# ElesionKyrie/Extreme-Video-Compression-With-Prediction-Using-Pre-trainded-Diffusion-Models-

Measured on AMD Instinct MI355X. Metric: decoded frames/sec (128x128x30) at q3, higher is better.
Workload: dtype f32

## Files before the change

extreme-video-compression-with-prediction-using-pre-trainded-diffusion-models-_amd/build.py:

```python
import os
import shutil
import subprocess
import sys
from concurrent.futures import ThreadPoolExecutor

HERE = os.path.dirname(os.path.abspath(__file__))
CSRC = os.path.join(HERE, "csrc")
LIBDIR = os.path.join(HERE, "lib")
OBJDIR = os.path.join(HERE, "build")
INCLUDE = os.path.join(os.path.dirname(HERE), "include")
HIP_SOURCES = ["conv_igemm.hip", "attention.hip", "norm.hip", "fir.hip", "elementwise.hip", "gdn.hip", "stride2.hip", "lpips.hip", "i3d.hip", "frames.hip", "noise.hip", "yuv.hip", "rate.hip", "ssim.hip", "metric.hip", "inception.hip", "resample.hip", "tile.hip", "api.hip"]
ARCH = "gfx950"


def _newer(target, deps):
    if not os.path.exists(target):
        return True
    t = os.path.getmtime(target)
    return any(os.path.getmtime(d) > t for d in deps)


def _run(cmd):
    r = subprocess.run(cmd, capture_output=True, text=True)
    if r.returncode != 0:
        raise RuntimeError("build failed: %s\n%s\n%s" % (" ".join(cmd), r.stdout, r.stderr))


def hipcc_path():
    for c in (os.environ.get("HIPCC"), shutil.which("hipcc"), "/opt/rocm/bin/hipcc"):
        if c and os.path.exists(c):
            return c
    raise RuntimeError("hipcc not found (ROCm toolchain required to build libevc_hip.so)")


def build(force=False, verbose=False):
    os.makedirs(LIBDIR, exist_ok=True)
    os.makedirs(OBJDIR, exist_ok=True)
    headers = [os.path.join(INCLUDE, h) for h in ("evc_hip.h", "evc_rans.h")]
    hipcc = hipcc_path()
    flags = ["--offload-arch=" + ARCH, "-O3", "-std=c++17", "-fPIC", "-I", INCLUDE]
    flags += os.environ.get("EVC_HIPCC_FLAGS", "").split()

    def compile_one(src):
        s = os.path.join(CSRC, src)
        o = os.path.join(OBJDIR, src.replace(".hip", ".o"))
        if force or _newer(o, [s] + headers):
            if verbose:
                print("hipcc", src, flush=True)
            _run([hipcc] + flags + ["-c", s, "-o", o])
        return o

    with ThreadPoolExecutor(max_workers=min(6, len(HIP_SOURCES))) as ex:
        objs = list(ex.map(compile_one, HIP_SOURCES))
    hip_so = os.path.join(LIBDIR, "libevc_hip.so")
    if force or _newer(hip_so, objs):
        _run([hipcc, "--offload-arch=" + ARCH, "-shared", "-fPIC", "-o", hip_so] + objs)
    rans_src = os.path.join(CSRC, "rans.cpp")
    rans_so = os.path.join(LIBDIR, "libevc_rans.so")
    if force or _newer(rans_so, [rans_src] + headers):
        _run([shutil.which("g++") or "g++", "-O2", "-std=c++17", "-fPIC", "-shared", "-Wall", "-I", INCLUDE,
              rans_src, "-o", rans_so])
# ... 6 lines not shown
```

extreme-video-compression-with-prediction-using-pre-trainded-diffusion-models-_amd/csrc/conv_igemm.hip:

```cpp
#include <hip/hip_runtime.h>
#include <stdint.h>
#include <stdio.h>
#include "../../include/evc_hip.h"

typedef float f32x16 __attribute__((ext_vector_type(16)));
typedef __attribute__((address_space(3))) void lds_void;
typedef const __attribute__((address_space(1))) void glb_void;

#ifndef EVC_CONV_TAIL
#define EVC_CONV_TAIL 1
#endif
#ifndef EVC_CONV_TM1
#define EVC_CONV_TM1 1
#endif
#ifndef EVC_SPLIT_WIDE_TILES
#define EVC_SPLIT_WIDE_TILES 1
#endif

#ifndef EVC_SPLIT_INTERLEAVE
#define EVC_SPLIT_INTERLEAVE 5
#endif

namespace {

constexpr int BM_MAX = 128;
constexpr int KC = 16;

constexpr int MODE_PLAIN = 0, MODE_AFFINE = 1, MODE_AFFINE_SILU = 2, MODE_SILU = 3, MODE_RELU = 4;

struct ConvK {
    const float* src0; const float* src1; int C0; int C1; int ld0; int ld1;
    const float* coef_a; const float* coef_s;
    const float* w; const float* bias; const float* res; int ld_res;
    float out_scale; int act_out;
    float* out; int ld_out;
    int B, H, W, Co, CoPad, KH, KW;
    int M, HW, nchunk, nsteps, steps_per_split, splits;
    float* ws;
    float* stats;
    const float* w_hdr;
    const unsigned* in_bound;
    int tail_first, tail_splits, tail_sps, tail_rows;
    int cut_chunk;
    const float* x2_src0; const float* x2_src1; int x2_C0, x2_C1, x2_ld0, x2_ld1;
    const char* x2_w;
    const float* x2_hdr;
    const unsigned* x2_bound;
    int bound_stride, generic_epi;
};

__device__ __forceinline__ float bound_scale(unsigned bits) {
    const float b = sqrtf(__uint_as_float(bits));
    if (!(b < 3.0e38f)) return __builtin_nanf("");
    return b > 0.f ? ldexpf(1.0f, 6 - ilogbf(b)) : 1.0f;
}
__device__ __forceinline__ int bound_index(const ConvK& p, int m) { return p.bound_stride ? min(m, p.M - 1) / p.HW : 0; }
__device__ __forceinline__ float in_scale(const ConvK& p, int m) {
    if (!p.in_bound) return 1.0f;
    return bound_scale(p.in_bound[bound_index(p, m)]);
}

__device__ __forceinline__ float silu_f(float v) { return v * __builtin_amdgcn_rcpf(1.0f + __expf(-v)); }

__device__ __forceinline__ float act_fn(float v, int act) {
    if (act == EVC_ACT_SILU) return silu_f(v);
    if (act == EVC_ACT_RELU) return v < 0.f ? 0.f : v;
    return v;
}

template <int MODE>
__device__ __forceinline__ float4 transform(float4 v, const float4& a, const float4& s, bool ok) {
    if (MODE == MODE_AFFINE || MODE == MODE_AFFINE_SILU) {
        v.x = v.x * a.x + s.x; v.y = v.y * a.y + s.y; v.z = v.z * a.z + s.z; v.w = v.w * a.w + s.w;
    }
    if (MODE == MODE_AFFINE_SILU || MODE == MODE_SILU) {
        v.x = silu_f(v.x); v.y = silu_f(v.y); v.z = silu_f(v.z); v.w = silu_f(v.w);
    }
    if (MODE == MODE_RELU) {
// ... 248 lines not shown
        issue_loads(buf ^ 1);

        const float* Ab = As + buf * BM * KC + a_rd;
        const float* Wb = Ws + buf * BN * KC + w_rd;
        float4 a0[TM], b0[TN], a1[TM], b1[TN];
#pragma unroll
        for (int i = 0; i < TM; ++i) a0[i] = *reinterpret_cast<const float4*>(Ab + i * 32 * KC + rd0);
#pragma unroll
        for (int j = 0; j < TN; ++j) b0[j] = *reinterpret_cast<const float4*>(Wb + j * 32 * KC + rd0);
#pragma unroll
        for (int i = 0; i < TM; ++i) a1[i] = *reinterpret_cast<const float4*>(Ab + i * 32 * KC + rd1);
#pragma unroll
        for (int j = 0; j < TN; ++j) b1[j] = *reinterpret_cast<const float4*>(Wb + j * 32 * KC + rd1);
        mfma_group<TM, TN>(acc, a0, b0);
        __builtin_amdgcn_sched_barrier(0);
        store_a(buf ^ 1);
        mfma_group<TM, TN>(acc, a1, b1);
        __syncthreads();
    }

    conv_epilogue<TM, TN>(p, acc, m0, n0, split, wm, wn, l31, half);
}

typedef __bf16 bf16x8 __attribute__((ext_vector_type(8)));
typedef _Float16 f16x8 __attribute__((ext_vector_type(8)));

__device__ __forceinline__ void split3_bf16(const float4& v0, const float4& v1, bf16x8& p1, bf16x8& p2, bf16x8& p3) {
    const float x[8] = {v0.x, v0.y, v0.z, v0.w, v1.x, v1.y, v1.z, v1.w};
#pragma unroll
    for (int j = 0; j < 8; ++j) {
        const __bf16 a = (__bf16)x[j];
        const float r = x[j] - (float)a;
        const __bf16 b = (__bf16)r;
        p1[j] = a; p2[j] = b; p3[j] = (__bf16)(r - (float)b);
    }
}

constexpr float F16_ACT_SCALE = 8.0f;

__device__ __forceinline__ void split2_f16(const float4& v0, const float4& v1, float xscale, f16x8& p1, f16x8& p2) {
    const float x[8] = {v0.x, v0.y, v0.z, v0.w, v1.x, v1.y, v1.z, v1.w};
#pragma unroll
    for (int j = 0; j < 8; ++j) {
        const float v = x[j] * xscale;
        const _Float16 a = (_Float16)v;
        p1[j] = a; p2[j] = (_Float16)(v - (float)a);
    }
}

template <int NP> struct Split;
template <> struct Split<3> {
    typedef bf16x8 vec;
    static constexpr int NTERM = 6;
    static __device__ __forceinline__ constexpr int qa(int t) { return t == 0 ? 2 : (t == 1 || t == 3) ? 1 : 0; }
    static __device__ __forceinline__ constexpr int qb(int t) { return t == 2 ? 2 : (t == 1 || t == 4) ? 1 : 0; }
    static __device__ __forceinline__ f32x16 mfma(const vec& a, const vec& b, const f32x16& c) {
        return __builtin_amdgcn_mfma_f32_32x32x16_bf16(a, b, c, 0, 0, 0);
    }
    static __device__ __forceinline__ void split(const float4& v0, const float4& v1, float, vec (&pl)[3]) {
        split3_bf16(v0, v1, pl[0], pl[1], pl[2]);
    }
};
template <> struct Split<2> {
    typedef f16x8 vec;
    static constexpr int NTERM = 3;
    static __device__ __forceinline__ constexpr int qa(int t) { return t == 0 ? 1 : 0; }
    static __device__ __forceinline__ constexpr int qb(int t) { return t == 1 ? 1 : 0; }
    static __device__ __forceinline__ f32x16 mfma(const vec& a, const vec& b, const f32x16& c) {
        return __builtin_amdgcn_mfma_f32_32x32x16_f16(a, b, c, 0, 0, 0);
    }
    static __device__ __forceinline__ void split(const float4& v0, const float4& v1, float xscale, vec (&pl)[2]) {
        split2_f16(v0, v1, xscale, pl[0], pl[1]);
    }
};

template <int NP, int TM, int TN, int MODE>
__global__ __launch_bounds__(256, 2) void conv_splitn_kernel(ConvK p) {
    typedef Split<NP> SP;
    typedef typename SP::vec vec;
    constexpr int BM = 64 * TM;
    constexpr int BN = 64 * TN;
    constexpr int RB = 32;
    constexpr int NPIECE = NP * 2 * TN;
    constexpr int NWD = (NPIECE + 3) / 4;
    constexpr bool HAS_COEF = MODE == MODE_AFFINE || MODE == MODE_AFFINE_SILU;
    extern __shared__ __attribute__((aligned(16))) char smem_b[];
    char* const As = smem_b;
    char* const Ws = smem_b + 2 * NP * BM * RB;

    const int tid = threadIdx.x;
    const int lane = tid & 63;
    const int wave = __builtin_amdgcn_readfirstlane(tid >> 6);
    const int wm = wave >> 1, wn = wave & 1;
    const int l31 = lane & 31, half = lane >> 5;

    const int m0 = blockIdx.x * BM;
    const int n0 = blockIdx.y * BN;
// ... 1196 lines not shown
__global__ void conv_pack_split_kernel(const float* w, __bf16* packed, int Co, int CoPad, int Ci, int KH, int KW) {
    const int taps = KH * KW, nchunk = Ci / KC;
    const size_t total = (size_t)taps * nchunk * CoPad * KC;
    for (size_t i = (size_t)blockIdx.x * blockDim.x + threadIdx.x; i < total; i += (size_t)gridDim.x * blockDim.x) {
        const int k = (int)(i % KC);
        size_t t = i / KC;
        const int co = (int)(t % CoPad); t /= CoPad;
        const int chunk = (int)(t % nchunk);
        const int tap = (int)(t / nchunk);
        float v = 0.f;
        if (co < Co) v = w[((size_t)co * Ci + chunk * KC + k) * taps + tap];
        const __bf16 a = (__bf16)v;
        const float r = v - (float)a;
        const __bf16 b = (__bf16)r;
        const __bf16 c = (__bf16)(r - (float)b);
        const int pos = (((k >> 3) ^ ((co >> 3) & 1)) << 3) | (k & 7);
        const size_t base = (size_t)(tap * nchunk + chunk) * 3 * CoPad * KC;
        packed[base + ((size_t)0 * CoPad + co) * KC + pos] = a;
        packed[base + ((size_t)1 * CoPad + co) * KC + pos] = b;
        packed[base + ((size_t)2 * CoPad + co) * KC + pos] = c;
    }
}

constexpr int F16_HDR_BYTES = 256;

__global__ void conv_absmax_kernel(const float* w, size_t n, unsigned* out_bits) {
    float m = 0.f;
    for (size_t i = (size_t)blockIdx.x * blockDim.x + threadIdx.x; i < n; i += (size_t)gridDim.x * blockDim.x)
        m = fmaxf(m, fabsf(w[i]));
    for (int o = 32; o > 0; o >>= 1) m = fmaxf(m, __shfl_xor(m, o));
    if ((threadIdx.x & 63) == 0 && m > 0.f) atomicMax(out_bits, __float_as_uint(m));
}

__device__ __forceinline__ float f16_weight_scale(unsigned max_bits) {
    const float mx = __uint_as_float(max_bits);
    if (!(mx > 0.f) || !isfinite(mx)) return 1.0f;
    return ldexpf(1.0f, 14 - ilogbf(mx));
}

__global__ void conv_pack_f16_kernel(const float* w, char* packed, int Co, int CoPad, int Ci, int KH, int KW) {
    const int taps = KH * KW, nchunk = Ci / KC;
    const size_t total = (size_t)taps * nchunk * CoPad * KC;
    float* hdr = reinterpret_cast<float*>(packed);
    const float sw = f16_weight_scale(reinterpret_cast<const unsigned*>(packed)[2]);
    _Float16* body = reinterpret_cast<_Float16*>(packed + F16_HDR_BYTES);
    if (blockIdx.x == 0 && threadIdx.x == 0) { hdr[0] = 1.0f / (F16_ACT_SCALE * sw); hdr[1] = sw; }
    for (size_t i = (size_t)blockIdx.x * blockDim.x + threadIdx.x; i < total; i += (size_t)gridDim.x * blockDim.x) {
// ... 585 lines not shown
```

extreme-video-compression-with-prediction-using-pre-trainded-diffusion-models-_amd/lib.py:

```python
import ctypes
import math
import os
from ctypes import POINTER, c_char_p, c_double, c_float, c_int, c_int32, c_longlong, c_uint, c_uint8, c_ulonglong, c_void_p

import numpy as np
import torch

HERE = os.path.dirname(os.path.abspath(__file__))
HIP_SO = os.path.join(HERE, "lib", "libevc_hip.so")
if os.environ.get("EVC_HIP_SO"):
    HIP_SO = os.path.abspath(os.environ["EVC_HIP_SO"])
RANS_SO = os.path.join(HERE, "lib", "libevc_rans.so")

ACT_NONE, ACT_SILU, ACT_RELU = 0, 1, 2
ARITH_F32, ARITH_BF16X6, ARITH_F16X3 = 0, 1, 2
_ARITH_NAMES = {"f32": ARITH_F32, "bf16x6": ARITH_BF16X6, "f16x3": ARITH_F16X3}
_ARITH_DTYPES = {ARITH_F32: torch.float32, ARITH_BF16X6: torch.bfloat16, ARITH_F16X3: torch.float16}


def _arith_policy():
    name = os.environ.get("EVC_CONV_ARITH", "f16x3").lower()
    if name not in _ARITH_NAMES:
        raise ValueError(f"EVC_CONV_ARITH must be one of {sorted(_ARITH_NAMES)}, got {name!r}")
    return _ARITH_NAMES[name]
# ... 13 lines not shown


class EvcKernelError(RuntimeError):
    pass


class ConvArgs(ctypes.Structure):
    _fields_ = [("src0", c_void_p), ("src1", c_void_p), ("C0", c_int), ("C1", c_int),
                ("ld0", c_int), ("ld1", c_int),
                ("coef_a", c_void_p), ("coef_s", c_void_p), ("act_in", c_int),
                ("w_packed", c_void_p), ("bias", c_void_p), ("res", c_void_p), ("ld_res", c_int),
                ("out_scale", c_float), ("act_out", c_int),
                ("out", c_void_p), ("ld_out", c_int),
                ("B", c_int), ("H", c_int), ("W", c_int), ("Co", c_int), ("KH", c_int), ("KW", c_int),
                ("splits", c_int), ("stats_out", c_void_p), ("arith", c_int), ("in_bound", c_void_p),
                ("x2_src0", c_void_p), ("x2_src1", c_void_p), ("x2_C0", c_int), ("x2_C1", c_int), ("x2_ld0", c_int),
                ("x2_ld1", c_int), ("x2_w_packed", c_void_p), ("x2_bound", c_void_p), ("invariant", c_int)]


class ConvPlan(ctypes.Structure):
    _fields_ = [("kernel", ctypes.c_char * 96), ("tile_m", c_int), ("tile_n", c_int), ("splits", c_int),
                ("steps_per_split", c_int), ("cut_chunk", c_int), ("tail_tiles", c_int), ("tail_splits", c_int),
                ("stats_runs", c_int), ("fused_1x1", c_int)]


class AttentionPlan(ctypes.Structure):
    _fields_ = [("kernel", ctypes.c_char * 64), ("waves", c_int), ("kparts", c_int), ("tiles_per_part", c_int),
                ("kv_planes", c_int), ("merge", c_int), ("short_seq", c_int),
                ("lds_bytes", c_longlong), ("parts_bytes", c_longlong), ("ws_bytes", c_longlong)]


HIP_SYMBOLS = {
    "evc_version": (c_char_p, []),
    "evc_arch": (c_char_p, []),
    "evc_device_ok": (c_int, []),
    "evc_clock_probe": (c_int, [c_void_p, c_int, c_void_p, c_void_p]),
    "evc_im2col_nchw_f32": (c_int, [c_void_p, c_void_p] + [c_int] * 9 + [c_void_p, c_void_p, c_void_p]),
    "evc_maxpool3s2_nhwc_f32": (c_int, [c_void_p, c_void_p, c_int, c_int, c_int, c_int, c_void_p]),
    "evc_lpips_layer_f32": (c_int, [c_void_p, c_void_p, c_void_p, c_void_p, c_int, c_int, c_int, c_int, c_void_p]),
    "evc_maxpool2d_nhwc_f32": (c_int, [c_void_p, c_void_p] + [c_int] * 7 + [c_void_p]),
    "evc_lpips_map_f32": (c_int, [c_void_p, c_void_p, c_void_p, c_void_p, c_int, c_int, c_int, c_void_p]),
    "evc_lpips_map_mean_f32": (c_int, [c_void_p, c_void_p, c_int, c_int, c_int, c_void_p]),
    "evc_lpips_upsample_add_f32": (c_int, [c_void_p, c_void_p] + [c_int] * 6 + [c_void_p]),
    "evc_i3d_stem_im2col_f32": (c_int, [c_void_p, c_void_p] + [c_int] * 17 + [c_void_p]),
    "evc_maxpool3d_same_nthwc_f32": (c_int, [c_void_p, c_void_p] + [c_int] * 11 + [c_void_p]),
    "evc_i3d_head_f32": (c_int, [c_void_p] * 4 + [c_int] * 6 + [c_void_p]),
# ... 39 lines not shown
    "evc_deconv5x5s2_f32": (c_int, [c_void_p, c_void_p, c_int, c_void_p, c_void_p, c_void_p] + [c_int] * 6 + [c_void_p]),
    "evc_conv5x5s2_workspace_bytes": (c_longlong, [c_int, c_int, c_int, c_int]),
    "evc_conv5x5s2_f32": (c_int, [c_void_p, c_int, c_void_p, c_int, c_void_p, c_void_p, c_void_p] + [c_int] * 6 + [c_void_p]),
    "evc_gdn_workspace_bytes": (c_longlong, [c_int, c_int, c_int, c_int]),
    "evc_gdn_f32": (c_int, [c_void_p, c_void_p, c_int, c_void_p, c_void_p, c_void_p, c_int, c_int, c_int, c_int, c_int,
                            c_int, c_void_p]),
    "evc_affine_act_nhwc_f32": (c_int, [c_void_p, c_void_p, c_void_p, c_void_p, c_int, c_int, c_int, c_int, c_int,
                                        c_int, c_void_p]),
    "evc_conv_co_pad": (c_int, [c_int]),
    "evc_conv_packed_floats": (c_longlong, [c_int, c_int, c_int, c_int]),
    "evc_conv_pack_weights_f32": (c_int, [c_void_p, c_void_p, c_int, c_int, c_int, c_int, c_void_p]),
    "evc_conv_packed_bytes": (c_longlong, [c_int, c_int, c_int, c_int, c_int]),
    "evc_conv_pack_weights": (c_int, [c_void_p, c_void_p, c_int, c_int, c_int, c_int, c_int, c_void_p]),
    "evc_conv_set_option": (c_int, [c_char_p, c_int]),
    "evc_spade_act_nhwc_f32": (c_int, [c_void_p, c_void_p, c_void_p, c_void_p, c_int, c_void_p, c_void_p, c_int, c_void_p,
                                       c_void_p, c_int, c_void_p, c_int, c_int, c_int, c_int, c_int, c_void_p]),
    "evc_conv_choose_splits": (c_int, [POINTER(ConvArgs)]),
    "evc_conv_kernel_name": (c_int, [POINTER(ConvArgs), c_char_p, c_int]),
    "evc_conv_fused_1x1_supported": (c_int, [POINTER(ConvArgs)]),
    "evc_conv_stats_splits": (c_int, [POINTER(ConvArgs)]),
    "evc_conv_workspace_bytes": (c_longlong, [POINTER(ConvArgs)]),
    "evc_conv2d_nhwc_f32": (c_int, [POINTER(ConvArgs), c_void_p, c_void_p]),
    "evc_conv2d_nhwc_profiled_f32": (c_int, [POINTER(ConvArgs), c_void_p, c_void_p, c_void_p, c_void_p]),
    "evc_attention_f32": (c_int, [c_void_p, c_void_p, c_void_p, c_int, c_void_p, c_int, c_int, c_int, c_int, c_int,
                                  c_float, c_void_p]),
    "evc_attention_workspace_bytes": (c_longlong, [c_int, c_int, c_int, c_int]),
    "evc_attention_set_option": (c_int, [c_char_p, c_int]),
    "evc_attention_plan_query": (c_int, [c_int, c_int, c_int, c_int, c_int, c_int, c_int, POINTER(AttentionPlan)]),
    "evc_attention_ws_f32": (c_int, [c_void_p, c_void_p, c_void_p, c_int, c_void_p, c_int, c_int, c_int, c_int, c_int,
                                     c_float, c_void_p, c_void_p]),
    "evc_frame_group_norm_f32": (c_int, [c_void_p] * 4 + [c_int] * 5 + [c_float, c_void_p]),
    "evc_frame_attention_f32": (c_int, [c_void_p, c_int, c_void_p, c_int] + [c_int] * 5 + [c_float, c_void_p]),
    "evc_frame_mix_f32": (c_int, [c_void_p] * 4 + [c_int] * 3 + [c_longlong, c_void_p]),
    "evc_frame_taps_f32": (c_int, [c_void_p, c_void_p] + [c_int] * 4 + [c_void_p]),
    "evc_ddpm_step_f32": (c_int, [c_void_p, c_void_p, c_void_p, c_longlong] + [c_float] * 5 + [c_int, c_void_p]),
    "evc_ddim_step_f32": (c_int, [c_void_p, c_void_p, c_longlong] + [c_float] * 4 + [c_int, c_void_p]),
    "evc_axpy_f32": (c_int, [c_void_p, c_void_p, c_void_p, c_longlong, c_float, c_void_p]),
    "evc_pndm_transfer_f32": (c_int, [c_void_p, c_void_p, c_void_p, c_longlong, c_float, c_float, c_float, c_int,
                                      c_void_p]),
    "evc_lincomb4_f32": (c_int, [c_void_p] * 5 + [c_longlong] + [c_float] * 4 + [c_void_p]),
    "evc_scale_clamp_f32": (c_int, [c_void_p, c_void_p, c_longlong, c_float, c_float, c_int, c_float, c_float,
                                    c_void_p]),
    "evc_gate_residual_f32": (c_int, [c_void_p, c_void_p, c_void_p, c_void_p, c_longlong, c_void_p]),
    "evc_elic_gather_params_f32": (c_int, [c_void_p] + [c_int] * 8 + [c_void_p, c_int, c_void_p, c_void_p,
                                                                       c_void_p]),
    "evc_elic_scatter_symbols_f32": (c_int, [c_void_p, c_void_p, c_void_p] + [c_int] * 7 + [c_void_p]),
# ... 669 lines not shown
                                 shape=(B, H, W, C0 + C1, Co, KH),
                                 call=dict(B=B, H=H, W=W, C0=C0, C1=C1, Co=Co, K=KH, coef=coef is not None, act_in=act_in,
                                           res=res is not None, out_scale=float(out_scale), bias=bias is not None,
                                           bound=in_bound is not None, arith=a.arith, ld_out=ldo,
                                           stats=bool(want_stats), x2=x2_ci, invariant=inv)))
    else:
        _check(L.evc_conv2d_nhwc_f32(ctypes.byref(a), ptr(ws), stream_ptr()), "evc_conv2d_nhwc_f32")
    result = out.t if isinstance(out, Cols) else out
    if want_stats:
        return result, (stats if stats is not None else chan_stats(result, invariant=inv))
    return result


def conv_fused_stats_splits(B, H, W, Ci, Co, KH, KW, splits=0, arith=None):
    a = conv_query_args(B, H, W, Ci, 0, Co, KH, KW, default_arith() if arith is None else arith, splits=splits)
    return hip_lib(require_device=False).evc_conv_stats_splits(ctypes.byref(a))


def conv_workspace_bytes(B, H, W, Ci, Co, KH, KW, splits=0, arith=None):
    a = conv_query_args(B, H, W, Ci, 0, Co, KH, KW, default_arith() if arith is None else arith, splits=splits)
    return hip_lib(require_device=False).evc_conv_workspace_bytes(ctypes.byref(a))


def attention_set_option(name, value):
    if hip_lib(require_device=False).evc_attention_set_option(name.encode(), int(value)) != 0:
        raise EvcKernelError(f"unknown attention option {name!r}")


ATTN_PROFILE = None


def attention_plan(B, heads, N, D, with_bounds=False, have_ws=None, invariant=False):
    L = hip_lib(require_device=False)
    if have_ws is None:
        nbytes = (L.evc_attention_invariant_workspace_bytes if invariant else L.evc_attention_workspace_bytes)(B, heads, N, D)
        have_ws = nbytes > 0
    out = AttentionPlan()
    _check(L.evc_attention_plan_query(B, heads, N, D, int(bool(with_bounds)), int(bool(have_ws)), int(bool(invariant)),
                                      ctypes.byref(out)), "evc_attention_plan_query")
    return dict(kernel=out.kernel.decode(), waves=out.waves, kparts=out.kparts, tiles_per_part=out.tiles_per_part,
                kv_planes=bool(out.kv_planes), merge=bool(out.merge), short_seq=bool(out.short_seq),
                lds_bytes=out.lds_bytes, parts_bytes=out.parts_bytes, ws_bytes=out.ws_bytes)


def attention(qkv, C, heads, out=None, bounds=None, invariant=False, ws=None):
    L = hip_lib()
# ... 536 lines not shown
```

extreme-video-compression-with-prediction-using-pre-trainded-diffusion-models-_amd/scorenet.py:

```python
import math
from types import SimpleNamespace

import numpy as np
import torch

from . import lib as L

FIR_K = np.outer([1, 3, 3, 1], [1, 3, 3, 1]).astype(np.float32)
FIR_K /= FIR_K.sum()
INV_SQRT2 = float(np.float32(1.0) / np.sqrt(np.float32(2.0)))


def num_groups(ch):
    g = min(ch // 4, 32)
    while ch % g != 0:
        g -= 1
    return g


def dims_from_config(config):
    m, d = config.model, config.data
    return SimpleNamespace(ngf=m.ngf, ch_mult=list(m.ch_mult), num_res_blocks=m.num_res_blocks,
                           attn_resolutions=list(m.attn_resolutions), n_head_channels=m.n_head_channels,
                           image_size=d.image_size, channels=d.channels, num_frames=d.num_frames,
# ... 492 lines not shown
        else:
            torch.cuda.current_stream().wait_event(done)
        if fuse:
            x2 = (xs, None, e["w2"], xbound) if xs is not None else (x.t, s1, e["w2"], xbound)
            return self._act(*self._conv(h1.t, e["w1"], m["cout"], 3, 3, bias=e["b12"], coef=coef1, act_in=L.ACT_SILU,
                                       out_scale=INV_SQRT2, want_stats=True, x2=x2))
        if self.preactivate:
            h1a = L.affine_act(h1.t, coef1, L.ACT_SILU)
            return self._act(*self._conv(h1a, e["w1"], m["cout"], 3, 3, bias=e["b1"], res=xs, out_scale=INV_SQRT2,
                                       want_stats=True))
        return self._act(*self._conv(h1.t, e["w1"], m["cout"], 3, 3, bias=e["b1"], coef=coef1, act_in=L.ACT_SILU,
                                   res=xs, out_scale=INV_SQRT2, want_stats=True))

    def _attn(self, i, m, x):
        e = self.w[i]
        B, H, W, C = x.t.shape
        hd = self.d.n_head_channels
        heads = 1 if C < hd else C // hd
        coef = self._gn([x.stats()], H * W, num_groups(C), 1e-6, mode=1, gamma=e["gamma"], beta=e["beta"],
                           site=self._site("attn_norm", i))
        qkvb = self._bound_slot(3)
        if qkvb is None:
            obound = None
            qkv = self._conv(x.t, e["wqkv"], 3 * C, 1, 1, bias=e["bqkv"], coef=coef)
        else:
            qkv, qst = self._conv(x.t, e["wqkv"], 3 * C, 1, 1, bias=e["bqkv"], coef=coef, want_stats=True)
            self._mbound(qst, 0, C, qkvb, site=self._site("attn_qkv", i))
            obound = _f16_only(e["wo"], qkvb.view(B, 3)[:, 2].contiguous() if self.batch_invariant else qkvb[2:3])
        o = self._attention(qkv.view(B, H * W, 3 * C), C, heads, bounds=None if i in self._attn_f32 else qkvb)
        return self._act(*self._conv(o.view(B, H, W, C), e["wo"], C, 1, 1, bias=e["bo"], res=x.t,
                                   out_scale=INV_SQRT2, want_stats=True, in_bound=obound))

    @torch.no_grad()
    def forward_rows(self, x, rows, cond=None):
        if self.batch_invariant and self._demoted:
            raise ValueError("batch-invariant mode does not combine with demoted sites (range recovery)")
        return self._forward_rows(x, rows, cond)

    def _forward_rows(self, x, rows, cond=None):
        d = self.d
        prog = self.program
        B, _, H, W = x.shape
        self._bound_batch = B if self.batch_invariant else 1
        nb = 256 * self._bound_batch
        if self._f16_raw:
            if torch.cuda.is_current_stream_capturing():
                self._bounds = torch.empty(nb, device=self.device, dtype=torch.int32)
            else:
                key = torch.cuda.current_stream().cuda_stream
                self._bounds = self._bounds_by_stream.get(key)
                if self._bounds is None or self._bounds.numel() != nb:
                    self._bounds = self._bounds_by_stream[key] = torch.empty(nb, device=self.device, dtype=torch.int32)
            self._bounds.zero_()
            self._bound_next = 0
# ... 120 lines not shown
```

include/evc_hip.h:

```cpp
#ifndef EVC_HIP_H
#define EVC_HIP_H

#ifdef __cplusplus
extern "C" {
#endif

#define EVC_OK 0
#define EVC_EINVAL (-1)
#define EVC_EUNSUPPORTED (-2)
#define EVC_ELAUNCH (-3)

#define EVC_ACT_NONE 0
#define EVC_ACT_SILU 1
#define EVC_ACT_RELU 2

#define EVC_ARITH_F32 0
#define EVC_ARITH_BF16X6 1
#define EVC_ARITH_F16X3 2

const char* evc_version(void);
const char* evc_arch(void);
int evc_device_ok(void);

int evc_clock_probe(unsigned long long* out2, int spin_us, const unsigned* stop, void* stream);
// ... 73 lines not shown
int evc_conv_stats_splits(const evc_conv_args* a);
long long evc_conv_workspace_bytes(const evc_conv_args* a);
int evc_conv2d_nhwc_f32(const evc_conv_args* a, float* ws, void* stream);

#define EVC_INVARIANT_REF_BATCH 9
int evc_invariant_plan_revision(void);
typedef struct {
    char kernel[96];
    int tile_m, tile_n, splits, steps_per_split, cut_chunk, tail_tiles, tail_splits, stats_runs, fused_1x1;
} evc_conv_plan;
int evc_conv_plan_query(const evc_conv_args* a, evc_conv_plan* out);
int evc_gn_coeffs_bound_sample_f32(const float* part0, int nsplit0, int C0, const float* part1, int nsplit1, int C1, int B,
                                   int HW, int groups, float eps, int mode, const float* gamma, const float* beta,
                                   const float* ss, int ss_ld, const int* row, float* coef_a, float* coef_s,
                                   unsigned* bound_bits, unsigned* events, unsigned* site_events, int site, void* stream);
int evc_moments_bound_sample_f32(const float* part, int nsplit, int C, int c_begin, int c_count, int n_ranges, int B,
                                 unsigned* bound_bits, unsigned* events, unsigned* site_events, int site, void* stream);
long long evc_attention_invariant_workspace_bytes(int B, int heads, int N, int D);
int evc_attention_invariant_f32(const float* q, const float* k, const float* v, int ld_qkv, float* out, int ld_out, int B,
                                int heads, int N, int D, float scale, const unsigned* bounds, float* ws, void* stream);

int evc_conv2d_nhwc_profiled_f32(const evc_conv_args* a, float* ws, void* stream, void* ev_start, void* ev_conv_end);

int evc_attention_f32(const float* q, const float* k, const float* v, int ld_qkv, float* out, int ld_out, int B,
                      int heads, int N, int D, float scale, void* stream);
long long evc_attention_workspace_bytes(int B, int heads, int N, int D);
int evc_attention_set_option(const char* name, int value);
int evc_attention_ws_f32(const float* q, const float* k, const float* v, int ld_qkv, float* out, int ld_out, int B,
                         int heads, int N, int D, float scale, float* ws, void* stream);

int evc_attention_f16x3_f32(const float* q, const float* k, const float* v, int ld_qkv, float* out, int ld_out, int B,
                            int heads, int N, int D, float scale, const unsigned* bounds, float* ws, void* stream);

typedef struct {
    char kernel[64];
    int waves, kparts, tiles_per_part, kv_planes, merge, short_seq;
    long long lds_bytes, parts_bytes, ws_bytes;
} evc_attention_plan;
int evc_attention_plan_query(int B, int heads, int N, int D, int with_bounds, int have_ws, int invariant,
                             evc_attention_plan* out);

int evc_frame_group_norm_f32(const float* x, float* y, const float* gamma, const float* beta, int B, int N, int HW, int C,
                             int groups, float eps, void* stream);
int evc_frame_attention_f32(const float* qkv, int ld_qkv, float* out, int ld_out, int B, int N, int HW, int C, int heads,
                            float scale, void* stream);
int evc_frame_mix_f32(const float* x, float* y, const float* w, const float* bias, int B, int N, int M, long long inner,
// ... 112 lines not shown
```

Before: 37.24.

## Add dedicated split-f16 MFMA GEMM kernel for attention 1x1 projections

Adds a specialized NHWC GEMM kernel for the 1x1 qkv and output projections in attention blocks. It uses split-f16 MFMA with register-prefetched weights, swizzled double-buffered LDS activations and a fused affine/bias/residual/stats epilogue. The goal is to avoid the overhead of the general implicit-GEMM conv path (split-K, workspace, tail handling) for these plain GEMMs. It falls back to the conv path for unsupported shapes or configurations, and it shares the split helpers moved into a common header.

```diff
diff --git a/extreme-video-compression-with-prediction-using-pre-trainded-diffusion-models-_amd/build.py b/extreme-video-compression-with-prediction-using-pre-trainded-diffusion-models-_amd/build.py
--- a/extreme-video-compression-with-prediction-using-pre-trainded-diffusion-models-_amd/build.py
+++ b/extreme-video-compression-with-prediction-using-pre-trainded-diffusion-models-_amd/build.py
@@ -9,7 +9,7 @@
 LIBDIR = os.path.join(HERE, "lib")
 OBJDIR = os.path.join(HERE, "build")
 INCLUDE = os.path.join(os.path.dirname(HERE), "include")
-HIP_SOURCES = ["conv_igemm.hip", "attention.hip", "norm.hip", "fir.hip", "elementwise.hip", "gdn.hip", "stride2.hip", "lpips.hip", "i3d.hip", "frames.hip", "noise.hip", "yuv.hip", "rate.hip", "ssim.hip", "metric.hip", "inception.hip", "resample.hip", "tile.hip", "api.hip"]
+HIP_SOURCES = ["conv_igemm.hip", "nin_gemm.hip", "attention.hip", "norm.hip", "fir.hip", "elementwise.hip", "gdn.hip", "stride2.hip", "lpips.hip", "i3d.hip", "frames.hip", "noise.hip", "yuv.hip", "rate.hip", "ssim.hip", "metric.hip", "inception.hip", "resample.hip", "tile.hip", "api.hip"]
 ARCH = "gfx950"
 
 
@@ -37,6 +37,7 @@
     os.makedirs(LIBDIR, exist_ok=True)
     os.makedirs(OBJDIR, exist_ok=True)
     headers = [os.path.join(INCLUDE, h) for h in ("evc_hip.h", "evc_rans.h")]
+    headers += [os.path.join(CSRC, h) for h in sorted(os.listdir(CSRC)) if h.endswith(".h")]
     hipcc = hipcc_path()
     flags = ["--offload-arch=" + ARCH, "-O3", "-std=c++17", "-fPIC", "-I", INCLUDE]
     flags += os.environ.get("EVC_HIPCC_FLAGS", "").split()
diff --git a/extreme-video-compression-with-prediction-using-pre-trainded-diffusion-models-_amd/csrc/conv_igemm.hip b/extreme-video-compression-with-prediction-using-pre-trainded-diffusion-models-_amd/csrc/conv_igemm.hip
--- a/extreme-video-compression-with-prediction-using-pre-trainded-diffusion-models-_amd/csrc/conv_igemm.hip
+++ b/extreme-video-compression-with-prediction-using-pre-trainded-diffusion-models-_amd/csrc/conv_igemm.hip
@@ -2,8 +2,8 @@
 #include <stdint.h>
 #include <stdio.h>
 #include "../../include/evc_hip.h"
-
-typedef float f32x16 __attribute__((ext_vector_type(16)));
+#include "split_mfma.h"
+
 typedef __attribute__((address_space(3))) void lds_void;
 typedef const __attribute__((address_space(1))) void glb_void;
 
@@ -49,11 +49,6 @@
     int bound_stride, generic_epi;
 };
 
-__device__ __forceinline__ float bound_scale(unsigned bits) {
-    const float b = sqrtf(__uint_as_float(bits));
-    if (!(b < 3.0e38f)) return __builtin_nanf("");
-    return b > 0.f ? ldexpf(1.0f, 6 - ilogbf(b)) : 1.0f;
-}
 __device__ __forceinline__ int bound_index(const ConvK& p, int m) { return p.bound_stride ? min(m, p.M - 1) / p.HW : 0; }
 __device__ __forceinline__ float in_scale(const ConvK& p, int m) {
     if (!p.in_bound) return 1.0f;
@@ -348,57 +343,7 @@
     conv_epilogue<TM, TN>(p, acc, m0, n0, split, wm, wn, l31, half);
 }
 
-typedef __bf16 bf16x8 __attribute__((ext_vector_type(8)));
-typedef _Float16 f16x8 __attribute__((ext_vector_type(8)));
-
-__device__ __forceinline__ void split3_bf16(const float4& v0, const float4& v1, bf16x8& p1, bf16x8& p2, bf16x8& p3) {
-    const float x[8] = {v0.x, v0.y, v0.z, v0.w, v1.x, v1.y, v1.z, v1.w};
-#pragma unroll
-    for (int j = 0; j < 8; ++j) {
-        const __bf16 a = (__bf16)x[j];
-        const float r = x[j] - (float)a;
-        const __bf16 b = (__bf16)r;
-        p1[j] = a; p2[j] = b; p3[j] = (__bf16)(r - (float)b);
-    }
-}
-
-constexpr float F16_ACT_SCALE = 8.0f;
-
-__device__ __forceinline__ void split2_f16(const float4& v0, const float4& v1, float xscale, f16x8& p1, f16x8& p2) {
-    const float x[8] = {v0.x, v0.y, v0.z, v0.w, v1.x, v1.y, v1.z, v1.w};
-#pragma unroll
-    for (int j = 0; j < 8; ++j) {
-        const float v = x[j] * xscale;
-        const _Float16 a = (_Float16)v;
-        p1[j] = a; p2[j] = (_Float16)(v - (float)a);
-    }
-}
-
-template <int NP> struct Split;
-template <> struct Split<3> {
-    typedef bf16x8 vec;
-    static constexpr int NTERM = 6;
-    static __device__ __forceinline__ constexpr int qa(int t) { return t == 0 ? 2 : (t == 1 || t == 3) ? 1 : 0; }
-    static __device__ __forceinline__ constexpr int qb(int t) { return t == 2 ? 2 : (t == 1 || t == 4) ? 1 : 0; }
-    static __device__ __forceinline__ f32x16 mfma(const vec& a, const vec& b, const f32x16& c) {
-        return __builtin_amdgcn_mfma_f32_32x32x16_bf16(a, b, c, 0, 0, 0);
-    }
-    static __device__ __forceinline__ void split(const float4& v0, const float4& v1, float, vec (&pl)[3]) {
-        split3_bf16(v0, v1, pl[0], pl[1], pl[2]);
-    }
-};
-template <> struct Split<2> {
-    typedef f16x8 vec;
-    static constexpr int NTERM = 3;
-    static __device__ __forceinline__ constexpr int qa(int t) { return t == 0 ? 1 : 0; }
-    static __device__ __forceinline__ constexpr int qb(int t) { return t == 1 ? 1 : 0; }
-    static __device__ __forceinline__ f32x16 mfma(const vec& a, const vec& b, const f32x16& c) {
-        return __builtin_amdgcn_mfma_f32_32x32x16_f16(a, b, c, 0, 0, 0);
-    }
-    static __device__ __forceinline__ void split(const float4& v0, const float4& v1, float xscale, vec (&pl)[2]) {
-        split2_f16(v0, v1, xscale, pl[0], pl[1]);
-    }
-};
+
 
 template <int NP, int TM, int TN, int MODE>
 __global__ __launch_bounds__(256, 2) void conv_splitn_kernel(ConvK p) {
@@ -1641,7 +1586,6 @@
     }
 }
 
-constexpr int F16_HDR_BYTES = 256;
 
 __global__ void conv_absmax_kernel(const float* w, size_t n, unsigned* out_bits) {
     float m = 0.f;
diff --git a/extreme-video-compression-with-prediction-using-pre-trainded-diffusion-models-_amd/csrc/nin_gemm.hip b/extreme-video-compression-with-prediction-using-pre-trainded-diffusion-models-_amd/csrc/nin_gemm.hip
--- /dev/null
+++ b/extreme-video-compression-with-prediction-using-pre-trainded-diffusion-models-_amd/csrc/nin_gemm.hip
@@ -0,0 +1,283 @@
+#include <hip/hip_runtime.h>
+#include <stdint.h>
+#include <stdio.h>
+#include "../../include/evc_hip.h"
+#include "split_mfma.h"
+
+namespace {
+
+struct NinK {
+    const float* x; const float* coef_a; const float* coef_s; const unsigned* in_bound;
+    const char* w;
+    const float* w_hdr;
+    const float* bias; const float* res; float out_scale;
+    float* out; float* stats;
+    int M, HW, K, Co, nstage;
+};
+
+template <int TM, int TN, bool RES, bool STATS>
+__device__ __forceinline__ void nin_epilogue(const NinK& p, f32x16 (&acc)[TM][TN], int m0, int n0, int wm, int wn, int l31,
+                                             int half) {
+    const float ascale = p.w_hdr[0] / (p.in_bound ? bound_scale(p.in_bound[0]) : 1.0f);
+    const float oscale = p.out_scale;
+    const int mw = m0 + wm * 32 * TM + 4 * half;
+    const int cw = n0 + wn * 32 * TN + l31;
+#pragma unroll
+    for (int j = 0; j < TN; ++j) {
+        const int co = cw + j * 32;
+        const float bias = p.bias ? p.bias[co] : 0.f;
+        float st_sum = 0.f, st_sq = 0.f;
+#pragma unroll
+        for (int i = 0; i < TM; ++i) {
+            const int mb = mw + i * 32;
+            float rv[16];
+#pragma unroll
+            for (int r = 0; r < 16; ++r) rv[r] = 0.f;
+            if (RES) {
+                const float* rp = p.res + (size_t)mb * p.Co + co;
+#pragma unroll
+                for (int r = 0; r < 16; ++r) rv[r] = rp[(size_t)((r & 3) + 8 * (r >> 2)) * p.Co];
+            }
+            float* o = p.out + (size_t)mb * p.Co + co;
+#pragma unroll
+            for (int r = 0; r < 16; ++r) {
+                float v = (acc[i][j][r] * ascale + bias + rv[r]) * oscale;
+                o[(size_t)((r & 3) + 8 * (r >> 2)) * p.Co] = v;
+                if (STATS) { st_sum += v; st_sq += v * v; }
+            }
+        }
+        if (STATS) {
+            st_sum += __shfl_xor(st_sum, 32);
+            st_sq += __shfl_xor(st_sq, 32);
+            if (half == 0) {
+                float* sp = p.stats + ((size_t)(m0 / (32 * TM) + wm) * p.Co + co) * 2;
+                sp[0] = st_sum; sp[1] = st_sq;
+            }
+        }
+    }
+}
+
+__device__ __forceinline__ void pin(float4& v) { asm volatile("" : "+v"(v.x), "+v"(v.y), "+v"(v.z), "+v"(v.w)); }
+
+template <int TM, int TN, bool AFFINE>
+__global__ __launch_bounds__(256, 2) void nin_gemm_kernel(NinK p) {
+    typedef Split<2> SP;
+    typedef SP::vec vec;
+    constexpr int BM = 64 * TM;
+    constexpr int BN = 64 * TN;
+    constexpr int RB = 32;
+    constexpr int NJ = 2 * TM;
+    constexpr int PLANE = BM * RB, STEP = 2 * PLANE, BUF = 4 * STEP;
+    extern __shared__ __attribute__((aligned(16))) char smem_nin[];
+
+    const int tid = threadIdx.x;
+    const int lane = tid & 63;
+    const int wave = __builtin_amdgcn_readfirstlane(tid >> 6);
+    const int wm = wave >> 1, wn = wave & 1;
+    const int l31 = lane & 31, half = lane >> 5;
+    const int m0 = blockIdx.x * BM;
+    const int n0 = blockIdx.y * BN;
+
+    const int pc = tid & 7, sc = pc >> 1, skh = pc & 1, srow = tid >> 3;
+    const char* const xg = reinterpret_cast<const char*>(p.x + (size_t)m0 * p.K) + ((size_t)srow * p.K + pc * 8) * 4;
+    const unsigned xstep = 32u * (unsigned)p.K * 4u;
+    const size_t cofs = (size_t)(m0 / p.HW) * p.K + pc * 8;
+    int a_wr[NJ];
+#pragma unroll
+    for (int j = 0; j < NJ; ++j) {
+        const int row = srow + 32 * j;
+        a_wr[j] = sc * STEP + (row ^ sc) * RB + 16 * (skh ^ ((row >> 3) & 1));
+    }
+    const int swz = 16 * (half ^ ((l31 >> 3) & 1));
+    const int a_rd = wm * 32 * TM * RB + swz;
+    const char* const wg = p.w + (size_t)(n0 + wn * 32 * TN + l31) * RB + swz;
+    const unsigned wplane = (unsigned)p.Co * RB;
+
+    const float xscale = F16_ACT_SCALE * (p.in_bound ? bound_scale(p.in_bound[0]) : 1.0f);
+
+    float4 areg[NJ][2], ca[2], cs[2];
+    vec breg[4][TN][2];
+    auto load_a = [&](int s) {
+        const char* src = xg + (size_t)s * 256;
+#pragma unroll
+        for (int j = 0; j < NJ; ++j) {
+            areg[j][0] = *reinterpret_cast<const float4*>(src + j * xstep);
+            areg[j][1] = *reinterpret_cast<const float4*>(src + j * xstep + 16);
+        }
+        if (AFFINE) {
+            const float* a = p.coef_a + cofs + s * 64;
+            const float* c = p.coef_s + cofs + s * 64;
+            ca[0] = *reinterpret_cast<const float4*>(a); ca[1] = *reinterpret_cast<const float4*>(a + 4);
+            cs[0] = *reinterpret_cast<const float4*>(c); cs[1] = *reinterpret_cast<const float4*>(c + 4);
+        }
+    };
+    auto load_b = [&](int s, int c) {
+        const char* src = wg + (size_t)(s * 4 + c) * 2 * wplane;
+#pragma unroll
+        for (int j = 0; j < TN; ++j)
+#pragma unroll
+            for (int q = 0; q < 2; ++q) breg[c][j][q] = *reinterpret_cast<const vec*>(src + q * wplane + j * 32 * RB);
+    };
+    auto affine = [&](float4 v, const float4& a, const float4& s) {
+        if (AFFINE) { v.x = v.x * a.x + s.x; v.y = v.y * a.y + s.y; v.z = v.z * a.z + s.z; v.w = v.w * a.w + s.w; }
+        return v;
+    };
+    auto store_a = [&](int buf) {
+        char* A = smem_nin + buf * BUF;
+#pragma unroll
+        for (int j = 0; j < NJ; ++j) {
+            vec pl[2];
+            pin(areg[j][0]); pin(areg[j][1]);
+            SP::split(affine(areg[j][0], ca[0], cs[0]), affine(areg[j][1], ca[1], cs[1]), xscale, pl);
+            *reinterpret_cast<vec*>(A + a_wr[j]) = pl[0];
+            *reinterpret_cast<vec*>(A + a_wr[j] + PLANE) = pl[1];
+        }
+    };
+
+    f32x16 acc[TM][TN];
+#pragma unroll
+    for (int i = 0; i < TM; ++i)
+#pragma unroll
+        for (int j = 0; j < TN; ++j)
+#pragma unroll
+            for (int r = 0; r < 16; ++r) acc[i][j][r] = 0.f;
+
+    load_a(0);
+#pragma unroll
+    for (int c = 0; c < 4; ++c) load_b(0, c);
+    store_a(0);
+    __syncthreads();
+
+    for (int s = 0; s < p.nstage; ++s) {
+        const int buf = s & 1;
+        const int sn = min(s + 1, p.nstage - 1);
+        load_a(sn);
+        __builtin_amdgcn_sched_barrier(0);
+        const char* Ab = smem_nin + buf * BUF + a_rd;
+#pragma unroll
+        for (int c = 0; c < 4; ++c) {
+            vec a[TM][2];
+#pragma unroll
+            for (int q = 0; q < 2; ++q)
+#pragma unroll
+                for (int i = 0; i < TM; ++i)
+                    a[i][q] = *reinterpret_cast<const vec*>(Ab + c * STEP + q * PLANE + ((i * 32 + l31) ^ c) * RB);
+#pragma unroll
+            for (int t = 0; t < SP::NTERM; ++t)
+#pragma unroll
+                for (int i = 0; i < TM; ++i)
+#pragma unroll
+                    for (int j = 0; j < TN; ++j) acc[i][j] = SP::mfma(a[i][SP::qa(t)], breg[c][j][SP::qb(t)], acc[i][j]);
+            __builtin_amdgcn_sched_barrier(0);
+            load_b(sn, c);
+            __builtin_amdgcn_sched_barrier(0);
+            if (c == 1) store_a(buf ^ 1);
+        }
+        __syncthreads();
+    }
+
+    if (p.res) {
+        if (p.stats) nin_epilogue<TM, TN, true, true>(p, acc, m0, n0, wm, wn, l31, half);
+        else nin_epilogue<TM, TN, true, false>(p, acc, m0, n0, wm, wn, l31, half);
+    } else {
+        if (p.stats) nin_epilogue<TM, TN, false, true>(p, acc, m0, n0, wm, wn, l31, half);
+        else nin_epilogue<TM, TN, false, false>(p, acc, m0, n0, wm, wn, l31, half);
+    }
+}
+
+
+constexpr int NIN_SLOTS = 512;
+
+constexpr int NIN_CONV_KEEPS = 256;
+
+struct NinLaunch {
+    int tm, tn, runs;
+    bool affine;
+    dim3 grid;
+    size_t lds;
+    NinK k;
+};
+
+bool nin_pick_tile(long long M, int K, int N, int HW, int& tm, int& tn) {
+    (void)K;
+    static const int cand[3][2] = {{2, 2}, {2, 1}, {1, 1}};
+    long long best = -1;
+    for (const auto& c : cand) {
+        const int bm = 64 * c[0], bn = 64 * c[1];
+        if (HW % bm != 0 || N % bn != 0) continue;
+        const long long wgs = (M / bm) * (N / bn);
+        const long long cost = ((wgs + NIN_SLOTS - 1) / NIN_SLOTS) * (bm * bn + 64 * 64);
+        if (best < 0 || cost < best) { best = cost; tm = c[0]; tn = c[1]; }
+    }
+    return best >= 0;
+}
+
+int nin_resolve(const evc_nin_args* a, NinLaunch& p) {
+    if (!a || !a->x || !a->w_packed || !a->out) return EVC_EINVAL;
+    if (a->B <= 0 || a->H <= 0 || a->W <= 0 || a->Ci <= 0 || a->Co <= 0) return EVC_EINVAL;
+    if (a->arith != EVC_ARITH_F16X3) return EVC_EUNSUPPORTED;
+    if (a->x1) return EVC_EUNSUPPORTED;
+    if (a->Ci % 64 != 0 || a->Co % 64 != 0) return EVC_EUNSUPPORTED;
+    if (a->act_out != EVC_ACT_NONE) return EVC_EUNSUPPORTED;
+    const bool coef = a->coef_a && a->coef_s;
+    if ((a->coef_a != nullptr) != (a->coef_s != nullptr)) return EVC_EINVAL;
+    if (coef == (a->in_bound != nullptr)) return EVC_EUNSUPPORTED;
+    const long long HW = (long long)a->H * a->W, M = HW * a->B;
+    if (M * a->Ci * 4 >= (1LL << 32) || M * a->Co >= (1LL << 31) || HW >= (1LL << 31)) return EVC_EUNSUPPORTED;
+    if (a->tile) {
+        p.tm = a->tile / 10; p.tn = a->tile % 10;
+        if ((a->tile != 22 && a->tile != 21 && a->tile != 11) || HW % (64 * p.tm) != 0 || a->Co % (64 * p.tn) != 0) return EVC_EUNSUPPORTED;
+    } else {
+        if (a->Co % 192 == 0 && HW % 128 == 0 && (M / 128) * (a->Co / 192) >= NIN_CONV_KEEPS) return EVC_EUNSUPPORTED;
+        if (!nin_pick_tile(M, a->Ci, a->Co, (int)HW, p.tm, p.tn)) return EVC_EUNSUPPORTED;
+    }
+    p.affine = coef;
+    p.runs = (int)HW / (32 * p.tm);
+    p.grid = dim3((unsigned)(M / (64 * p.tm)), (unsigned)(a->Co / (64 * p.tn)));
+    p.lds = (size_t)2 * 4 * 2 * 64 * p.tm * 32;
+    NinK& k = p.k;
+    k.M = (int)M; k.HW = (int)HW; k.K = a->Ci; k.Co = a->Co; k.nstage = a->Ci / 64;
+    return EVC_OK;
+}
+
+int nin_kernel_name(const NinLaunch& p, char* buf, int n) {
+    return snprintf(buf, n, "nin_gemm_kernel<%d, %d, %s>", p.tm, p.tn, p.affine ? "true" : "false");
+}
+
+template <int TM, int TN>
+void nin_launch(const NinLaunch& p, hipStream_t st) {
+    if (p.affine) hipLaunchKernelGGL((nin_gemm_kernel<TM, TN, true>), p.grid, dim3(256), p.lds, st, p.k);
+    else hipLaunchKernelGGL((nin_gemm_kernel<TM, TN, false>), p.grid, dim3(256), p.lds, st, p.k);
+}
+
+}
+
+extern "C" int evc_nin_gemm_supported(const evc_nin_args* a) {
+    NinLaunch p;
+    return nin_resolve(a, p) == EVC_OK ? 1 : 0;
+}
+
+extern "C" int evc_nin_gemm_plan_query(const evc_nin_args* a, evc_nin_plan* out) {
+    NinLaunch p;
+    const int rc = !out ? EVC_EINVAL : nin_resolve(a, p);
+    if (rc != EVC_OK) return rc;
+    nin_kernel_name(p, out->kernel, (int)sizeof(out->kernel));
+    out->tile_m = 64 * p.tm; out->tile_n = 64 * p.tn; out->stages = p.k.nstage; out->stats_runs = p.runs;
+    return EVC_OK;
+}
+
+extern "C" int evc_nin_gemm_f32(const evc_nin_args* a, void* stream) {
+    NinLaunch p;
+    const int rc = nin_resolve(a, p);
+    if (rc != EVC_OK) return rc;
+    NinK& k = p.k;
+    k.x = a->x; k.coef_a = a->coef_a; k.coef_s = a->coef_s; k.in_bound = a->in_bound;
+    k.w_hdr = a->w_packed;
+    k.w = reinterpret_cast<const char*>(a->w_packed) + F16_HDR_BYTES;
+    k.bias = a->bias; k.res = a->res; k.out_scale = a->out_scale; k.out = a->out; k.stats = a->stats_out;
+    hipStream_t st = (hipStream_t)stream;
+    if (p.tm == 2 && p.tn == 2) nin_launch<2, 2>(p, st);
+    else if (p.tm == 2) nin_launch<2, 1>(p, st);
+    else nin_launch<1, 1>(p, st);
+    return hipGetLastError() == hipSuccess ? EVC_OK : EVC_ELAUNCH;
+}
diff --git a/extreme-video-compression-with-prediction-using-pre-trainded-diffusion-models-_amd/csrc/split_mfma.h b/extreme-video-compression-with-prediction-using-pre-trainded-diffusion-models-_amd/csrc/split_mfma.h
--- /dev/null
+++ b/extreme-video-compression-with-prediction-using-pre-trainded-diffusion-models-_amd/csrc/split_mfma.h
@@ -0,0 +1,67 @@
+#pragma once
+#include <hip/hip_runtime.h>
+
+namespace {
+
+typedef float f32x16 __attribute__((ext_vector_type(16)));
+
+__device__ __forceinline__ float bound_scale(unsigned bits) {
+    const float b = sqrtf(__uint_as_float(bits));
+    if (!(b < 3.0e38f)) return __builtin_nanf("");
+    return b > 0.f ? ldexpf(1.0f, 6 - ilogbf(b)) : 1.0f;
+}
+
+typedef __bf16 bf16x8 __attribute__((ext_vector_type(8)));
+typedef _Float16 f16x8 __attribute__((ext_vector_type(8)));
+
+__device__ __forceinline__ void split3_bf16(const float4& v0, const float4& v1, bf16x8& p1, bf16x8& p2, bf16x8& p3) {
+    const float x[8] = {v0.x, v0.y, v0.z, v0.w, v1.x, v1.y, v1.z, v1.w};
+#pragma unroll
+    for (int j = 0; j < 8; ++j) {
+        const __bf16 a = (__bf16)x[j];
+        const float r = x[j] - (float)a;
+        const __bf16 b = (__bf16)r;
+        p1[j] = a; p2[j] = b; p3[j] = (__bf16)(r - (float)b);
+    }
+}
+
+constexpr float F16_ACT_SCALE = 8.0f;
+constexpr int F16_HDR_BYTES = 256;
+
+__device__ __forceinline__ void split2_f16(const float4& v0, const float4& v1, float xscale, f16x8& p1, f16x8& p2) {
+    const float x[8] = {v0.x, v0.y, v0.z, v0.w, v1.x, v1.y, v1.z, v1.w};
+#pragma unroll
+    for (int j = 0; j < 8; ++j) {
+        const float v = x[j] * xscale;
+        const _Float16 a = (_Float16)v;
+        p1[j] = a; p2[j] = (_Float16)(v - (float)a);
+    }
+}
+
+template <int NP> struct Split;
+template <> struct Split<3> {
+    typedef bf16x8 vec;
+    static constexpr int NTERM = 6;
+    static __device__ __forceinline__ constexpr int qa(int t) { return t == 0 ? 2 : (t == 1 || t == 3) ? 1 : 0; }
+    static __device__ __forceinline__ constexpr int qb(int t) { return t == 2 ? 2 : (t == 1 || t == 4) ? 1 : 0; }
+    static __device__ __forceinline__ f32x16 mfma(const vec& a, const vec& b, const f32x16& c) {
+        return __builtin_amdgcn_mfma_f32_32x32x16_bf16(a, b, c, 0, 0, 0);
+    }
+    static __device__ __forceinline__ void split(const float4& v0, const float4& v1, float, vec (&pl)[3]) {
+        split3_bf16(v0, v1, pl[0], pl[1], pl[2]);
+    }
+};
+template <> struct Split<2> {
+    typedef f16x8 vec;
+    static constexpr int NTERM = 3;
+    static __device__ __forceinline__ constexpr int qa(int t) { return t == 0 ? 1 : 0; }
+    static __device__ __forceinline__ constexpr int qb(int t) { return t == 1 ? 1 : 0; }
+    static __device__ __forceinline__ f32x16 mfma(const vec& a, const vec& b, const f32x16& c) {
+        return __builtin_amdgcn_mfma_f32_32x32x16_f16(a, b, c, 0, 0, 0);
+    }
+    static __device__ __forceinline__ void split(const float4& v0, const float4& v1, float xscale, vec (&pl)[2]) {
+        split2_f16(v0, v1, xscale, pl[0], pl[1]);
+    }
+};
+
+}
diff --git a/extreme-video-compression-with-prediction-using-pre-trainded-diffusion-models-_amd/lib.py b/extreme-video-compression-with-prediction-using-pre-trainded-diffusion-models-_amd/lib.py
--- a/extreme-video-compression-with-prediction-using-pre-trainded-diffusion-models-_amd/lib.py
+++ b/extreme-video-compression-with-prediction-using-pre-trainded-diffusion-models-_amd/lib.py
@@ -59,6 +59,17 @@
     _fields_ = [("kernel", ctypes.c_char * 96), ("tile_m", c_int), ("tile_n", c_int), ("splits", c_int),
                 ("steps_per_split", c_int), ("cut_chunk", c_int), ("tail_tiles", c_int), ("tail_splits", c_int),
                 ("stats_runs", c_int), ("fused_1x1", c_int)]
+
+
+class NinArgs(ctypes.Structure):
+    _fields_ = [("x", c_void_p), ("x1", c_void_p), ("Ci", c_int), ("Co", c_int), ("coef_a", c_void_p), ("coef_s", c_void_p),
+                ("in_bound", c_void_p), ("w_packed", c_void_p), ("arith", c_int), ("bias", c_void_p), ("res", c_void_p),
+                ("out_scale", c_float), ("act_out", c_int), ("out", c_void_p), ("stats_out", c_void_p),
+                ("B", c_int), ("H", c_int), ("W", c_int), ("tile", c_int)]
+
+
+class NinPlan(ctypes.Structure):
+    _fields_ = [("kernel", ctypes.c_char * 64), ("tile_m", c_int), ("tile_n", c_int), ("stages", c_int), ("stats_runs", c_int)]
 
 
 class AttentionPlan(ctypes.Structure):
@@ -144,6 +155,9 @@
     "evc_conv_workspace_bytes": (c_longlong, [POINTER(ConvArgs)]),
     "evc_conv2d_nhwc_f32": (c_int, [POINTER(ConvArgs), c_void_p, c_void_p]),
     "evc_conv2d_nhwc_profiled_f32": (c_int, [POINTER(ConvArgs), c_void_p, c_void_p, c_void_p, c_void_p]),
+    "evc_nin_gemm_supported": (c_int, [POINTER(NinArgs)]),
+    "evc_nin_gemm_plan_query": (c_int, [POINTER(NinArgs), POINTER(NinPlan)]),
+    "evc_nin_gemm_f32": (c_int, [POINTER(NinArgs), c_void_p]),
     "evc_attention_f32": (c_int, [c_void_p, c_void_p, c_void_p, c_int, c_void_p, c_int, c_int, c_int, c_int, c_int,
                                   c_float, c_void_p]),
     "evc_attention_workspace_bytes": (c_longlong, [c_int, c_int, c_int, c_int]),
@@ -859,6 +873,55 @@
     return hip_lib(require_device=False).evc_conv_workspace_bytes(ctypes.byref(a))
 
 
+NIN_PROFILE = None
+
+
+def nin_query_args(B, H, W, Ci, Co, arith=ARITH_F16X3, coef=False, bound=None, two_sources=False, act_out=ACT_NONE, tile=0):
+    d = c_void_p(16)
+    bound = (not coef) if bound is None else bound
+    return NinArgs(x=d, x1=d if two_sources else None, Ci=Ci, Co=Co, coef_a=d if coef else None, coef_s=d if coef else None,
+                   in_bound=d if bound else None, w_packed=d, arith=arith, out_scale=1.0, act_out=act_out, out=d,
+                   B=B, H=H, W=W, tile=tile)
+
+
+def nin_gemm_supported(B, H, W, Ci, Co, arith=ARITH_F16X3, coef=False, **kw):
+    a = nin_query_args(B, H, W, Ci, Co, arith, coef, **kw)
+    return bool(hip_lib(require_device=False).evc_nin_gemm_supported(ctypes.byref(a)))
+
+
+def nin_gemm_plan(B, H, W, Ci, Co, arith=ARITH_F16X3, coef=False, **kw):
+    out = NinPlan()
+    a = nin_query_args(B, H, W, Ci, Co, arith, coef, **kw)
+    _check(hip_lib(require_device=False).evc_nin_gemm_plan_query(ctypes.byref(a), ctypes.byref(out)), "evc_nin_gemm_plan_query")
+    return dict(kernel=out.kernel.decode(), tile=(out.tile_m, out.tile_n), stages=out.stages, stats_runs=out.stats_runs)
+
+
+def nin_gemm(x, w_packed, Co, bias=None, coef=None, res=None, out_scale=1.0, in_bound=None, want_stats=False, out=None,
+             tile=0):
+    L = hip_lib()
+    B, H, W, Ci = x.shape
+    assert x.is_contiguous() and x.dtype == torch.float32 and (res is None or (res.is_contiguous() and res.shape == (B, H, W, Co)))
+    if out is None:
+        out = torch.empty((B, H, W, Co), device=x.device, dtype=torch.float32)
+    assert out.is_contiguous() and out.shape == (B, H, W, Co)
+    ca, cs = coef if coef is not None else (None, None)
+    assert ca is None or (ca.shape == (B, Ci) and cs.shape == (B, Ci) and ca.is_contiguous() and cs.is_contiguous())
+    a = NinArgs(x=ptr(x), x1=None, Ci=Ci, Co=Co, coef_a=ptr(ca), coef_s=ptr(cs), in_bound=_word(in_bound),
+                w_packed=ptr(w_packed), arith=packed_arith(w_packed), bias=ptr(bias), res=ptr(res), out_scale=float(out_scale),
+                act_out=ACT_NONE, out=ptr(out), B=B, H=H, W=W, tile=tile)
+    plan = NinPlan()
+    _check(L.evc_nin_gemm_plan_query(ctypes.byref(a), ctypes.byref(plan)), "evc_nin_gemm_plan_query")
+    stats = None
+    if want_stats:
+        stats = torch.empty((B, plan.stats_runs, Co, 2), device=x.device, dtype=torch.float32)
+        a.stats_out = ptr(stats)
+    _check(L.evc_nin_gemm_f32(ctypes.byref(a), stream_ptr()), "evc_nin_gemm_f32")
+    if NIN_PROFILE is not None:
+        NIN_PROFILE.append(dict(kernel=plan.kernel.decode(), tile=(plan.tile_m, plan.tile_n), shape=(B, H, W, Ci, Co),
+                                coef=coef is not None, bound=in_bound is not None, res=res is not None, stats=bool(want_stats)))
+    return (out, stats) if want_stats else out
+
+
 def attention_set_option(name, value):
     if hip_lib(require_device=False).evc_attention_set_option(name.encode(), int(value)) != 0:
         raise EvcKernelError(f"unknown attention option {name!r}")
diff --git a/extreme-video-compression-with-prediction-using-pre-trainded-diffusion-models-_amd/scorenet.py b/extreme-video-compression-with-prediction-using-pre-trainded-diffusion-models-_amd/scorenet.py
--- a/extreme-video-compression-with-prediction-using-pre-trainded-diffusion-models-_amd/scorenet.py
+++ b/extreme-video-compression-with-prediction-using-pre-trainded-diffusion-models-_amd/scorenet.py
@@ -538,14 +538,26 @@
         qkvb = self._bound_slot(3)
         if qkvb is None:
             obound = None
-            qkv = self._conv(x.t, e["wqkv"], 3 * C, 1, 1, bias=e["bqkv"], coef=coef)
+            qkv = self._proj(x.t, e["wqkv"], 3 * C, e["bqkv"], coef=coef)
         else:
-            qkv, qst = self._conv(x.t, e["wqkv"], 3 * C, 1, 1, bias=e["bqkv"], coef=coef, want_stats=True)
+            qkv, qst = self._proj(x.t, e["wqkv"], 3 * C, e["bqkv"], coef=coef, want_stats=True)
             self._mbound(qst, 0, C, qkvb, site=self._site("attn_qkv", i))
             obound = _f16_only(e["wo"], qkvb.view(B, 3)[:, 2].contiguous() if self.batch_invariant else qkvb[2:3])
         o = self._attention(qkv.view(B, H * W, 3 * C), C, heads, bounds=None if i in self._attn_f32 else qkvb)
-        return self._act(*self._conv(o.view(B, H, W, C), e["wo"], C, 1, 1, bias=e["bo"], res=x.t,
-                                   out_scale=INV_SQRT2, want_stats=True, in_bound=obound))
+        return self._act(*self._proj(o.view(B, H, W, C), e["wo"], C, e["bo"], res=x.t, out_scale=INV_SQRT2, want_stats=True,
+                                     in_bound=obound))
+
+    nin_gemm = True
+
+    def _proj(self, x, w, Co, bias, coef=None, res=None, out_scale=1.0, want_stats=False, in_bound=None):
+        B, H, W, Ci = x.shape
+        plain = not self.batch_invariant and not self.SPADE and self.ARCH == "unetmore"
+        if self.nin_gemm and plain and L.packed_arith(w) == L.ARITH_F16X3 and \
+                L.nin_gemm_supported(B, H, W, Ci, Co, coef=coef is not None, bound=in_bound is not None):
+            return L.nin_gemm(x, w, Co, bias=bias, coef=coef, res=res, out_scale=out_scale, in_bound=in_bound,
+                              want_stats=want_stats)
+        return self._conv(x, w, Co, 1, 1, bias=bias, coef=coef, res=res, out_scale=out_scale, want_stats=want_stats,
+                          in_bound=in_bound)
 
     @torch.no_grad()
     def forward_rows(self, x, rows, cond=None):
diff --git a/include/evc_hip.h b/include/evc_hip.h
--- a/include/evc_hip.h
+++ b/include/evc_hip.h
@@ -119,6 +119,26 @@
 
 int evc_conv2d_nhwc_profiled_f32(const evc_conv_args* a, float* ws, void* stream, void* ev_start, void* ev_conv_end);
 
+typedef struct {
+    const float* x; const float* x1;
+    int Ci; int Co;
+    const float* coef_a; const float* coef_s;
+    const unsigned* in_bound;
+    const float* w_packed; int arith;
+    const float* bias; const float* res;
+    float out_scale; int act_out;
+    float* out; float* stats_out;
+    int B; int H; int W;
+    int tile;
+} evc_nin_args;
+typedef struct {
+    char kernel[64];
+    int tile_m, tile_n, stages, stats_runs;
+} evc_nin_plan;
+int evc_nin_gemm_supported(const evc_nin_args* a);
+int evc_nin_gemm_plan_query(const evc_nin_args* a, evc_nin_plan* out);
+int evc_nin_gemm_f32(const evc_nin_args* a, void* stream);
+
 int evc_attention_f32(const float* q, const float* k, const float* v, int ld_qkv, float* out, int ld_out, int B,
                       int heads, int N, int D, float scale, void* stream);
 long long evc_attention_workspace_bytes(int B, int heads, int N, int D);
```

Measured after the change: 37.72, median of 6. 1.01x the previous value.
